# samson6460/tf2_YOLO

Measured on AMD Instinct MI355X. Metric: images/sec training YOLOv3 416x416 bs=32/GPU, higher is better.
Workload: dtype f32-storage/fp16x2-mfma

## Files before the change

### include/yolo_hip.h

```cpp
#ifndef YOLO_HIP_H_
#define YOLO_HIP_H_

#include <stddef.h>
#include <stdint.h>

#ifdef __cplusplus
extern "C" {
#endif

typedef enum yolo_status {
  YOLO_OK = 0,
  YOLO_ERR_INVALID_ARG = -1,
  YOLO_ERR_LAUNCH = -2,
  YOLO_ERR_WORKSPACE = -3
} yolo_status;

enum { YOLO_ACT_LINEAR = 0, YOLO_ACT_LEAKY = 1, YOLO_ACT_MISH = 2 };
enum { YOLO_HEAD_V3 = 3, YOLO_HEAD_V2 = 2, YOLO_HEAD_V1 = 1, YOLO_HEAD_V4 = 4 };
enum { YOLO_NMS_HARD = 1, YOLO_NMS_SOFT = 2, YOLO_NMS_DIOU = 3 };

const char* yolo_last_error(void);
int yolo_abi_version(void);
int yolo_device_available(void);
int yolo_mfma_probe(const void* operands_f16, float* sink, int workgroups, int iters, double* flops_host, void* stream);

enum { YOLO_OPT_CONV_WIN = 0, YOLO_OPT_STAMPS = 1, YOLO_OPT_CONV_SK = 2, YOLO_OPT_CONV_PATCH = 5, YOLO_OPT_WGRAD_WIN = 6,
       YOLO_OPT_NMS_WALK = 7 ,
       YOLO_OPT_AB = 8  };
int yolo_set_option(int key, int value);
size_t yolo_conv_workspace_bytes(void);
int yolo_set_conv_workspace(void* p, size_t bytes, void* stream);
int yolo_set_debug_buffer(void* p, size_t bytes);

typedef struct yolo_conv_desc {
  int N, H, W, Cin;
  int Cout, kh, kw;
  int Ho, Wo;
  int sh, sw;
  int pad_t, pad_l;
} yolo_conv_desc;

#define YOLO_BN_STAT_SLOTS 64
#define YOLO_BN_RED_SLOTS 512
#define YOLO_SPLIT_BATCH_UNITS 4

int yolo_conv2d_fwd(const yolo_conv_desc* d, const float* x, const float* w,
                    const float* bias, float* y, double* stats, void* stream);
int yolo_conv2d_fwd_absmax(const yolo_conv_desc* d, const float* x, const float* w, const float* bias,
                           float* y, double* stats, unsigned* absmax, void* stream);

int yolo_conv2d_dgrad(const yolo_conv_desc* d, const float* dy, const float* wT,
                      float* dx, int accumulate, void* stream);

int yolo_conv2d_wgrad(const yolo_conv_desc* d, const float* x, const float* dy,
                      float* dw, float* dbias, void* stream);

int yolo_conv2d_wgrad_bias(const float* dy, long long P, int Cout, float* dbias, void* stream);

int yolo_filter_transpose(const float* w, float* wT, int Cout, int taps, int Cin, void* stream);

size_t yolo_planes_bytes(long long rows, int C);
int yolo_split_planes(const float* x, long long rows, int C, void* planes, void* stream);
int yolo_split_planes_padded(const float* x, long long rows, int C_src, int C, void* planes, void* stream);

int yolo_split_planes_batch(const void* jobs, int njobs, long long total_blocks, void* stream);
int yolo_filter_transpose_batch(const void* jobs, int njobs, long long total_blocks, void* stream);

int yolo_conv2d_fwd_planes(const yolo_conv_desc* d, const void* x_planes, const void* w_planes,
                           const float* bias, float* y, double* stats, unsigned* absmax, void* stream);
int yolo_conv2d_dgrad_planes(const yolo_conv_desc* d, const void* dy_planes, const void* wT_planes,
                             float* dx, int accumulate, void* stream);
enum { YOLO_EPI_NONE = 0, YOLO_EPI_AFFINE = 1, YOLO_EPI_AFFINE_LEAKY = 2, YOLO_EPI_AFFINE_MISH = 3 };
int yolo_conv2d_fwd_planes_epi(const yolo_conv_desc* d, const void* x_planes, const void* w_planes, const float* bias,
                               int epilogue, const float* scale, const float* shift, const float* residual, float* y,
                               unsigned* absmax, void* stream);
int yolo_split_planes_absmax(const float* x, long long rows, int C, const unsigned* absmax, const float* extra_bound,
                             void* planes, float* out_bound, void* stream);
#define YOLO_INFER_BOUND_WORDS 4096
int yolo_conv_pred_bound(const float* w, int Cout, int kdim, const float* scale, const float* shift, const float* bias,
                         float* pred2, void* stream);
int yolo_conv2d_fwd_infer_unit(const yolo_conv_desc* d, const void* x_planes, const void* w_planes, const float* bias,
                               int epilogue, const float* scale, const float* shift, const float* residual, float* y,
                               unsigned* absmax, const float* pred2, const void* in_bound, int in_n,
                               const void* residual_bound, int residual_n, void* out_planes, unsigned* out_words,
                               float* out_bound, int* out_n_host, void* stream);
int yolo_fold_bound(const void* words, int n, float* out_bound, void* stream);
int yolo_absmax_words(const float* x, long long n, unsigned* words, int* n_words_host, void* stream);
int yolo_stem_filter_prep(const float* w, const float* bias, float* wt, void* stream);
int yolo_stem_fwd_infer_unit(const yolo_conv_desc* d, const float* x, const float* wt, int epilogue, const float* scale,
                             const float* shift, const float* pred2, const void* in_bound, int in_n, float* y,
                             void* out_planes, unsigned* out_words, int* out_n_host, void* stream);
int yolo_split_planes_concat(const float* const* srcs_host, const int* channels_host, const float* const* bounds_host,
                             int nsrc, long long rows, void* planes, float* dst32, float* out_bound, void* stream);
int yolo_split_planes_concat_ex(const float* const* srcs_host, const int* channels_host, const float* const* bounds_host,
                                const int* bound_words_host, const int* upsample_host, int H, int W, int nsrc,
                                long long rows, void* planes, float* dst32, float* out_bound, void* stream);
int yolo_conv2d_fwd_head_unit(const yolo_conv_desc* d, const void* x_planes, const void* w_planes, const float* bias,
                              int A, int C, int version, const float* anchors, float* t, float* y, void* stream);
int yolo_conv2d_wgrad_planes(const yolo_conv_desc* d, const void* x_planes, const void* dy_planes,
                             float* dw, void* stream);

size_t yolo_wgrad_workspace_bytes(void);
int yolo_set_wgrad_workspace(void* p, size_t bytes);


int yolo_bn_stats(const float* x, long long P, int C, double* stats, void* stream);

int yolo_bn_finalize(double* stats, long long P, int C, const float* gamma, const float* beta,
                     float eps, float momentum, int unbiased_moving_var,
                     float* moving_mean, float* moving_var,
                     float* scale, float* shift, float* save_mean, float* save_invstd,
// ... 177 lines not shown
```

### tf2_yolo_amd/csrc/conv_args.hpp

```cpp
#pragma once
#include "common.hpp"

namespace yolo {

constexpr int MAX_TAPS = 49;

struct Tap {
  int oy, ox, woff;
};

struct ClassGeom {
  long long M;
  int Hg, Wg, ooy, oox, tap0, ntaps;
};

struct GatherConvArgs {
  const float* src;
  const float* wgt;
  const float* bias;
  float* dst;
  double* stats;
  unsigned* absmax;
  long long M;
  int N, Hs, Ws, Cs;
// ... 22 lines not shown
  const unsigned* pl_res_bound;
  int pl_in_n, pl_res_n;
  unsigned* pl_out_words;
  float* head_y;
  const float* head_anchors;
  int head_A, head_C;
  int sk_grid;
  int tile_order;
  float* sk_slabs;
  unsigned* sk_tickets;
  int split_parts;
  int ncls;
  ClassGeom cls[4];
  unsigned long long* stamps;
  const float* bwd_y;
  const float* bwd_scale;
  const float* bwd_shift;
  const float* bwd_mean;
  const float* bwd_invstd;
  float* bwd_part;
  unsigned* bwd_aux;
  int bwd_act;
  int bwd_nslots;
  int bwd_cap;
  Tap taps[MAX_TAPS];
};

#define YOLO_BNRED_CHECK(a)                                                                                          \
  if ((a).bwd_y != nullptr && (a).bwd_nslots > (a).bwd_cap) {                                                        \
    set_error("conv_dgrad(bn reduce): %d partial slots needed, room for %d", (a).bwd_nslots, (a).bwd_cap);           \
    return YOLO_ERR_INVALID_ARG;                                                                                     \
  }

__device__ __forceinline__ int xcd_remap(int bid, int nblocks) {
  const int xcd = bid & 7, idx = bid >> 3;
  const int q = nblocks >> 3, r = nblocks & 7;
  const int start = (xcd < r) ? xcd * (q + 1) : r * (q + 1) + (xcd - r) * q;
  return start + idx;
}


struct WgradArgs {
  const float* src;
  const float* dy;
  float* dw;
  long long M;
  int N, Hs, Ws, Cs;
  int Hg, Wg;
  int sy, sx;
  int Cout, ldw;
  int ntaps;
  int kw, pad_t, pad_l;
  int tiles_co, tiles_j;
  int nblocks;
  long long chunk;
  unsigned src_bytes, dy_bytes;
  int zero_blk_src, zero_blk_dy;
  float* slabs;
  int splits;
};

int launch_gather_split(GatherConvArgs& a, hipStream_t st);
bool gather_split_supported(const GatherConvArgs& a);
long long planes_bytes(long long rows, int C);
int launch_split_planes(const float* x, long long rows, int C, void* planes, hipStream_t st);
int launch_split_planes_absmax(const float* x, long long rows, int C, const unsigned* absmax, const float* extra_bound, int extra_n,
                               void* planes, float* out_bound, hipStream_t st);
int launch_split_planes_concat(const float* const* xs, const int* Cs, const float* const* bounds, int nsrc, long long rows,
                               void* planes, float* dst32, float* out_bound, hipStream_t st,
                               const int* bound_words = nullptr, const int* upsample = nullptr, int H = 0, int W = 0);
int launch_split_planes_padded(const float* x, long long rows, int Csrc, int C, void* planes, hipStream_t st);
int launch_split_planes_batch(const void* jobs, int njobs, long long total_blocks, hipStream_t st);
int launch_filter_transpose_batch(const void* jobs, int njobs, long long total_blocks, hipStream_t st);
int launch_gather_planes(GatherConvArgs& a, hipStream_t st);
bool conv_small_supported(const GatherConvArgs& a);
bool conv_small_head_supported(const GatherConvArgs& a);
int launch_conv_small(GatherConvArgs& a, hipStream_t st, int* nwg);
bool gather_planes_supported(const GatherConvArgs& a);
int conv_split_parts(const GatherConvArgs& a, long long nb, int bm, int min_cb, int idle_div);
int launch_split_reduce(GatherConvArgs& a, int bm, hipStream_t st);
float* conv_split_slabs();
int launch_conv_win(GatherConvArgs& a, int variant, hipStream_t st);
bool conv_win_supported(const GatherConvArgs& a);
enum { OPT_CONV_WIN = 0, OPT_STAMPS = 1, OPT_CONV_SK = 2, OPT_DBG = 3, OPT_TILE_ORDER = 4, OPT_CONV_PATCH = 5, OPT_WGRAD_WIN = 6, OPT_NMS_WALK = 7, OPT_EXP = 8, OPT_COUNT = 16 };
int set_conv_workspace(void* p, size_t bytes, hipStream_t st);
extern void* g_dbg_buf;
extern size_t g_dbg_bytes;
extern int g_opt[OPT_COUNT];
void init_options();
int launch_wgrad_planes(WgradArgs& a, hipStream_t st);
bool wgrad_planes_supported(const WgradArgs& a);
int launch_wgrad_win(WgradArgs& a, hipStream_t st);
bool wgrad_win_supported(const WgradArgs& a);
constexpr size_t WGRAD_WS_COLSUM_BYTES = 1 << 20;
void* wgrad_workspace(size_t* bytes);
bool stem_fwd_supported(const yolo_conv_desc* d);
struct StemEpiArgs {
  const float* scale;
  const float* shift;
  int act;
  void* planes;
  const float* pred;
  const unsigned* in_words;
  int in_n;
  unsigned* out_words;
};
bool stem_infer_supported(const yolo_conv_desc* d);
int launch_stem_filter_prep(const float* w, const float* bias, float* wt, hipStream_t st);
int launch_absmax_words(const float* x, long long n, unsigned* words, int* n_words, hipStream_t st);
int launch_stem_infer(const yolo_conv_desc* d, const float* x, const float* wt, float* y, const StemEpiArgs& e, int* out_n,
                      hipStream_t st);
size_t stem_bwd_scratch_bytes();
int launch_stem_bn_bwd_wgrad(const yolo_conv_desc* d, const float* y, const float* dout, const float* img, const float* scale,
                             const float* shift, const float* smean, const float* sinv, int act, const double* redsum,
                             float* dgamma, float* dbeta, float* dw, float* scratch, size_t scratch_bytes, hipStream_t st);
int launch_stem_fwd(const yolo_conv_desc* d, const float* x, const float* w, const float* bias, float* y, double* stats,
                    unsigned* absmax, hipStream_t st);
int launch_wgrad_split(WgradArgs& a, hipStream_t st);
bool wgrad_split_supported(const WgradArgs& a);

}
```

### tf2_yolo_amd/csrc/conv_wgrad_win.hip

```cpp
#include "planes.hpp"
#include <cstdlib>

namespace yolo {

typedef short ws16x4 __attribute__((ext_vector_type(4)));
typedef short ws16x8 __attribute__((ext_vector_type(8)));

constexpr int WW_CO = 128;
constexpr int WW_CI = 32;
constexpr int WW_STAGE_PX = 32;
constexpr int WW_TILE_FLOATS = WW_CO * 9 * WW_CI;

template <int RING, int KO = 0, int PF = 1>
__global__ __launch_bounds__(256, 2) void wgrad_win_kernel(const WgradArgs a) {
  constexpr int A_STAGE = 2 * 4 * PL_PLANES * 1024;
  constexpr int WIN_PLANE = RING * 64 + 64;
  constexpr int WIN_OFF = 2 * A_STAGE;
  constexpr unsigned RMASK = RING * 64 - 1;
  constexpr unsigned ZSLOT = RING * 64;

  extern __shared__ __attribute__((aligned(16))) unsigned char smem[];
  const unsigned lds_base = (unsigned)(size_t)smem;

  const int tid = threadIdx.x;
// ... 645 lines not shown
        acc[t][hf][1] = __builtin_amdgcn_mfma_f32_16x16x32_f16(ah[1], bh[cur], acc[t][hf][1], 0, 0, 0);
      }
      __builtin_amdgcn_sched_barrier(0);
      if (i == 17) {
#pragma unroll
        for (int r = 0; r < 2; ++r) {
          pb[r] = (pb[r] + WW_STAGE_PX * 64) & RMASK;
          int x = px[r] + adv_rem, y = py[r] + adv_rows;
          if (x >= W) {
            x -= W;
            ++y;
          }
          if (y >= H) y -= H;
          px[r] = x;
          py[r] = y;
        }
        __builtin_amdgcn_sched_barrier(0);
      }
    }
    asm volatile("s_waitcnt vmcnt(0)" ::: "memory");
    asm volatile("s_waitcnt lgkmcnt(0)" ::: "memory");
    __builtin_amdgcn_s_barrier();
  }

  const float unscale =
      reinterpret_cast<const float*>(reinterpret_cast<const unsigned char*>(a.dy) + a.dy_bytes - PL_HEADER)[2] *
      reinterpret_cast<const float*>(reinterpret_cast<const unsigned char*>(a.src) + a.src_bytes - PL_HEADER)[2];
  if (a.slabs != nullptr) {
    float* mine = a.slabs + (size_t)lid * WW_TILE_FLOATS;
#pragma unroll
    for (int t = 0; t < 9; ++t)
#pragma unroll
      for (int hf = 0; hf < 2; ++hf)
#pragma unroll
        for (int m = 0; m < 2; ++m)
          *reinterpret_cast<f32x4*>(mine + (((((wave * 9 + t) * 2 + hf) * 2 + m) * 64) + lane) * 4) = acc[t][hf][m];
    return;
  }
#pragma unroll
  for (int t = 0; t < 9; ++t)
#pragma unroll
    for (int hf = 0; hf < 2; ++hf) {
      const long long cj = (long long)t * a.Cs + ci0 + 16 * hf + (lane & 15);
#pragma unroll
      for (int m = 0; m < 2; ++m)
#pragma unroll
        for (int e = 0; e < 4; ++e) {
          const int co = co0 + wave * 32 + 16 * m + 4 * (lane >> 4) + e;
          atomicAdd(&a.dw[(long long)co * a.ldw + cj], acc[t][hf][m][e] * unscale);
        }
    }
}

__global__ __launch_bounds__(256) void wgrad_win16_reduce_kernel(const WgradArgs a) {
  constexpr int PER_TILE = WW_TILE_FLOATS / 4;
  const int tiles = a.tiles_co * a.tiles_j;
  const long long idx = (long long)blockIdx.x * 256 + threadIdx.x;
  const int tile = (int)(idx / PER_TILE);
  if (tile >= tiles) return;
  const int q = (int)(idx - (long long)tile * PER_TILE);
  const int lane = q & 63, piece = q >> 6;
  const int m = piece & 1, hf = (piece >> 1) & 1, t = (piece >> 2) % 9, wave = piece / 36;
  const int co = (tile % a.tiles_co) * WW_CO + wave * 32 + 16 * m + 4 * (lane >> 4);
  const long long cj = (long long)t * a.Cs + (tile / a.tiles_co) * WW_CI + 16 * hf + (lane & 15);
  const f32x4* sl = reinterpret_cast<const f32x4*>(a.slabs) + (size_t)tile * PER_TILE + q;
  const size_t sstride = (size_t)tiles * PER_TILE;
  f32x4 sum = {0.f, 0.f, 0.f, 0.f};
  int s = 0;
  for (; s + 8 <= a.splits; s += 8) {
    f32x4 v[8];
#pragma unroll
    for (int u = 0; u < 8; ++u) v[u] = __builtin_nontemporal_load(sl + (size_t)(s + u) * sstride);
#pragma unroll
    for (int u = 0; u < 8; ++u) sum = sum + v[u];
  }
  for (; s < a.splits; ++s) sum = sum + __builtin_nontemporal_load(sl + (size_t)s * sstride);
  const float unscale =
      reinterpret_cast<const float*>(reinterpret_cast<const unsigned char*>(a.dy) + a.dy_bytes - PL_HEADER)[2] *
      reinterpret_cast<const float*>(reinterpret_cast<const unsigned char*>(a.src) + a.src_bytes - PL_HEADER)[2];
#pragma unroll
  for (int e = 0; e < 4; ++e) a.dw[(long long)(co + e) * a.ldw + cj] += sum[e] * unscale;
}

bool wgrad_win_supported(const WgradArgs& a) {
  if (a.ntaps != 9 || a.kw != 3 || a.sy != 1 || a.sx != 1 || a.pad_t != 1 || a.pad_l != 1) return false;
  if (a.Hg != a.Hs || a.Wg != a.Ws) return false;
  if ((a.Cout % WW_CO) != 0 || (a.Cs % WW_CI) != 0 || a.ldw != 9 * a.Cs) return false;
  if (a.Ws < 4 || 2 * a.Ws + 81 > 512 || 32 / a.Ws + 2 > a.Hs) return false;
  if (a.M < 64 || a.M >= (1LL << 31) - 4096) return false;
  return true;
}

template <int RING, int KO, int PF = 1, bool M16 = false>
static int launch_ww(WgradArgs& a, hipStream_t st) {
  const void* kfn = M16 ? reinterpret_cast<const void*>(&wgrad_win16_kernel<RING, KO>)
                        : reinterpret_cast<const void*>(&wgrad_win_kernel<RING, KO, PF>);
  a.tiles_co = a.Cout / WW_CO;
  a.tiles_j = a.Cs / WW_CI;
  const long long tiles = (long long)a.tiles_co * a.tiles_j;
  constexpr size_t lds = 2 * (2 * 4 * PL_PLANES * 1024) + 2 * (RING * 64 + 64);
  static int resident = 0;
  static bool lds_from_zero = true;
  if (resident == 0) {
    int per_cu = 0, dev = 0, cus = 0;
    hipFuncAttributes fa{};
    if (hipFuncGetAttributes(&fa, kfn) != hipSuccess || fa.sharedSizeBytes != 0) lds_from_zero = false;
    (void)hipFuncSetAttribute(kfn, hipFuncAttributeMaxDynamicSharedMemorySize, (int)lds);
    if (hipOccupancyMaxActiveBlocksPerMultiprocessor(&per_cu, kfn, 256, lds) ==
            hipSuccess &&
        hipGetDevice(&dev) == hipSuccess && hipDeviceGetAttribute(&cus, hipDeviceAttributeMultiprocessorCount, dev) == hipSuccess)
      resident = per_cu * cus;
    if (resident <= 0) resident = 512;
  }
  if (!lds_from_zero) return 1;
  static const long long target_env = [] { const char* e = getenv("YOLO_WGRAD_WIN_TARGET"); return e ? atoll(e) : 0LL; }();
  const long long target = target_env > 0 ? target_env : (resident >= 2 ? resident / 2 : resident);
  long long splits = target / tiles;
  const long long max_splits = (a.M + 255) / 256;
  if (splits > max_splits) splits = max_splits;
  if (splits < 1) splits = 1;
  a.slabs = nullptr;
  static const bool det_env = [] { const char* e = getenv("YOLO_WGRAD_DETERMINISTIC"); return !(e && atoi(e) == 0); }();
  size_t ws_bytes = 0;
  void* ws = wgrad_workspace(&ws_bytes);
  if (det_env && ws != nullptr && ws_bytes > WGRAD_WS_COLSUM_BYTES) {
    const long long cap = (long long)((ws_bytes - WGRAD_WS_COLSUM_BYTES) / ((size_t)WW_TILE_FLOATS * 4));
    if (cap >= tiles) {
      if (tiles * splits > cap) splits = cap / tiles;
      a.slabs = reinterpret_cast<float*>(reinterpret_cast<unsigned char*>(ws) + WGRAD_WS_COLSUM_BYTES);
    }
  }
  long long chunk = (a.M + splits - 1) / splits;
  chunk = (chunk + 31) / 32 * 32;
  splits = (a.M + chunk - 1) / chunk;
  a.chunk = chunk;
  a.splits = (int)splits;
  a.nblocks = (int)(tiles * splits);
  if constexpr (M16) hipLaunchKernelGGL((wgrad_win16_kernel<RING, KO>), dim3((unsigned)a.nblocks), dim3(256), lds, st, a);
  else hipLaunchKernelGGL((wgrad_win_kernel<RING, KO, PF>), dim3((unsigned)a.nblocks), dim3(256), lds, st, a);
  if (int rc = check_launch("wgrad_win_kernel")) return rc;
  if (a.slabs != nullptr) {
    const long long pieces = tiles * (WW_TILE_FLOATS / 4);
    if constexpr (M16) hipLaunchKernelGGL(wgrad_win16_reduce_kernel, dim3((unsigned)((pieces + 255) / 256)), dim3(256), 0, st, a);
    else hipLaunchKernelGGL(wgrad_win_reduce_kernel, dim3((unsigned)((pieces + 255) / 256)), dim3(256), 0, st, a);
    return check_launch("wgrad_win_reduce_kernel");
  }
  return YOLO_OK;
}

static int launch_ww2(WgradArgs& a, hipStream_t st) {
  constexpr int RING = 256;
  const void* kfn = reinterpret_cast<const void*>(&wgrad_win2_kernel<RING>);
  a.tiles_co = a.Cout / WW_CO;
  a.tiles_j = a.Cs / WW_CI;
  const long long tiles = (long long)a.tiles_co * a.tiles_j;
  constexpr size_t half_bytes = 2 * (2 * 4 * PL_PLANES * 1024) + 2 * (RING * 64 + 64);
  constexpr size_t handover = (size_t)WW_TILE_FLOATS * 4;
  constexpr size_t lds = 2 * half_bytes > handover ? 2 * half_bytes : handover;
  static int resident = 0;
  static bool ok = true;
  if (resident == 0) {
    int per_cu = 0, dev = 0, cus = 0;
    hipFuncAttributes fa{};
    if (hipFuncGetAttributes(&fa, kfn) != hipSuccess || fa.sharedSizeBytes != 0) ok = false;
    if (hipFuncSetAttribute(kfn, hipFuncAttributeMaxDynamicSharedMemorySize, (int)lds) != hipSuccess) ok = false;
    if (hipOccupancyMaxActiveBlocksPerMultiprocessor(&per_cu, kfn, 512, lds) == hipSuccess && per_cu >= 1 &&
        hipGetDevice(&dev) == hipSuccess && hipDeviceGetAttribute(&cus, hipDeviceAttributeMultiprocessorCount, dev) == hipSuccess)
      resident = per_cu * cus;
    else
      ok = false;
    if (resident <= 0) resident = 256;
  }
  if (!ok) return 1;
  size_t ws_bytes = 0;
  void* ws = wgrad_workspace(&ws_bytes);
  static const bool det_env = [] { const char* e = getenv("YOLO_WGRAD_DETERMINISTIC"); return !(e && atoi(e) == 0); }();
  if (!det_env || ws == nullptr || ws_bytes <= WGRAD_WS_COLSUM_BYTES) return 1;
  long long splits = resident / tiles;
  const long long max_splits = (a.M + 511) / 512;
  if (splits > max_splits) splits = max_splits;
  if (splits < 1) splits = 1;
  const long long cap = (long long)((ws_bytes - WGRAD_WS_COLSUM_BYTES) / ((size_t)WW_TILE_FLOATS * 4));
  if (cap < tiles) return 1;
  if (tiles * splits > cap) splits = cap / tiles;
  a.slabs = reinterpret_cast<float*>(reinterpret_cast<unsigned char*>(ws) + WGRAD_WS_COLSUM_BYTES);
  long long chunk = (a.M + splits - 1) / splits;
  chunk = (chunk + 63) / 64 * 64;
  splits = (a.M + chunk - 1) / chunk;
  a.chunk = chunk;
  a.splits = (int)splits;
  a.nblocks = (int)(tiles * splits);
  hipLaunchKernelGGL((wgrad_win2_kernel<RING>), dim3((unsigned)a.nblocks), dim3(512), lds, st, a);
  if (int rc = check_launch("wgrad_win2_kernel")) return rc;
  const long long pieces = tiles * (WW_TILE_FLOATS / 4);
  hipLaunchKernelGGL(wgrad_win_reduce_kernel, dim3((unsigned)((pieces + 255) / 256)), dim3(256), 0, st, a);
  return check_launch("wgrad_win_reduce_kernel");
}

int launch_wgrad_win(WgradArgs& a, hipStream_t st) {
  const bool small = 2 * a.Ws + 81 <= 256;
  if (small && g_opt[OPT_WGRAD_WIN] == 4) {
    const int rc = launch_ww2(a, st);
    if (rc != 1) return rc;
  }
#ifdef YOLO_PLANES_KNOCKOUTS
  static const int ko = [] { const char* e = getenv("YOLO_WGRAD_KO"); return e ? atoi(e) : 0; }();
  if (small) switch (ko) {
      case 1: return launch_ww<256, 1>(a, st);
      case 2: return launch_ww<256, 2>(a, st);
      case 3: return launch_ww<256, 3>(a, st);
      case 4: return launch_ww<256, 4>(a, st);
      case 7: return launch_ww<256, 7>(a, st);
      case 8: return launch_ww<256, 8>(a, st);
      default: break;
    }
#endif
  if (small && g_opt[OPT_WGRAD_WIN] == 2) return launch_ww<256, 0, 2>(a, st);
  if (g_opt[OPT_WGRAD_WIN] == 3) return small ? launch_ww<256, 0, 1, true>(a, st) : launch_ww<512, 0, 1, true>(a, st);
  return small ? launch_ww<256, 0>(a, st) : launch_ww<512, 0>(a, st);
}

}
```

### tf2_yolo_amd/csrc/runtime.hip

```cpp
#include "conv_args.hpp"
#include <cstdlib>
#include <cstring>

namespace yolo {

static thread_local char g_err[512] = "";

void set_error(const char* fmt, ...) {
  va_list ap;
  va_start(ap, fmt);
  vsnprintf(g_err, sizeof(g_err), fmt, ap);
  va_end(ap);
}

int g_opt[OPT_COUNT];
void* g_dbg_buf = nullptr;
size_t g_dbg_bytes = 0;
static void options_from_env() {
  for (int i = 0; i < OPT_COUNT; ++i) g_opt[i] = 0;
  const char* e = getenv("YOLO_CONV_WIN");
  g_opt[OPT_CONV_WIN] = e ? atoi(e) : 1;
  e = getenv("YOLO_CONV_SK");
  g_opt[OPT_CONV_SK] = e ? atoi(e) : 1;
  e = getenv("YOLO_CONV_PATCH");
  g_opt[OPT_CONV_PATCH] = e ? atoi(e) : 1;
  e = getenv("YOLO_WGRAD_WIN");
  g_opt[OPT_WGRAD_WIN] = e ? atoi(e) : 1;
  e = getenv("YOLO_NMS_WALK");
  g_opt[OPT_NMS_WALK] = e ? atoi(e) : 0;
  e = getenv("YOLO_EXP");
  g_opt[OPT_EXP] = e ? atoi(e) : 0;
}
void init_options() {
  static bool done = false;
  if (done) return;
  done = true;
  options_from_env();
}

}

extern "C" int yolo_set_option(int key, int value) {
  yolo::init_options();
  if (key == -1) {
    yolo::options_from_env();
    return YOLO_OK;
  }
  if (key < 0 || key >= yolo::OPT_COUNT) {
    yolo::set_error("yolo_set_option: unknown key %d", key);
    return YOLO_ERR_INVALID_ARG;
  }
  yolo::g_opt[key] = value;
  return YOLO_OK;
}

extern "C" size_t yolo_conv_workspace_bytes(void) { return (size_t)(1 << 20) + (size_t)512 * 2 * 256 * 128 * 4; }

extern "C" int yolo_set_conv_workspace(void* p, size_t bytes, void* stream) {
  yolo::init_options();
  return yolo::set_conv_workspace(p, bytes, yolo::as_stream(stream));
}

extern "C" int yolo_set_debug_buffer(void* p, size_t bytes) {
  yolo::g_dbg_buf = p;
  yolo::g_dbg_bytes = bytes;
  return YOLO_OK;
}

extern "C" const char* yolo_last_error(void) { return yolo::g_err; }

extern "C" int yolo_abi_version(void) { return 5; }

#include <dlfcn.h>
namespace {
using nccl_allreduce_fn = int (*)(const void*, void*, size_t, int, int, void*, hipStream_t);
nccl_allreduce_fn find_nccl_allreduce() {
  void* f = dlsym(RTLD_DEFAULT, "ncclAllReduce");
  if (f == nullptr) {
    void* h = dlopen("librccl.so.1", RTLD_NOW | RTLD_GLOBAL);
    if (h == nullptr) h = dlopen("librccl.so", RTLD_NOW | RTLD_GLOBAL);
    if (h != nullptr) f = dlsym(h, "ncclAllReduce");
  }
  return reinterpret_cast<nccl_allreduce_fn>(f);
}
}

extern "C" int yolo_allreduce_bucket(void* rccl_comm, float* grads, long long count, void* stream) {
  YOLO_REQUIRE(rccl_comm != nullptr && grads != nullptr && count > 0, "allreduce_bucket: bad args");
  static nccl_allreduce_fn fn = find_nccl_allreduce();
  if (fn == nullptr) {
    yolo::set_error("allreduce_bucket: no RCCL in this process (ncclAllReduce not found, librccl.so not loadable)");
    return YOLO_ERR_LAUNCH;
  }
  constexpr int kNcclFloat = 7, kNcclSum = 0;
  const int rc = fn(grads, grads, (size_t)count, kNcclFloat, kNcclSum, rccl_comm, yolo::as_stream(stream));
  if (rc != 0) {
    yolo::set_error("allreduce_bucket: ncclAllReduce returned %d", rc);
    return YOLO_ERR_LAUNCH;
  }
  return YOLO_OK;
}

extern "C" int yolo_device_available(void) {
  int n = 0;
  if (hipGetDeviceCount(&n) != hipSuccess) return 0;
  return n > 0 ? 1 : 0;
}
```

### tf2_yolo_amd/ops.py

```python
import ctypes
from ctypes import byref, c_void_p

import torch

from . import _lib
from . import tape as _tape
from ._lib import ConvDesc, LossCfg, YoloHipError, check

BN_EPS = 1e-3
BN_MOMENTUM = 0.99
BN_STAT_SLOTS = 64
BN_RED_SLOTS = 512
SPLIT_BATCH_UNITS = 4


class KernelTimer:

    def __init__(self):
        self.pending = []

    def bracket(self, name, flops, launches, fn, layer=None):
        s, e = torch.cuda.Event(enable_timing=True), torch.cuda.Event(enable_timing=True)
        s.record()
        fn()
        e.record()
        self.pending.append((name, flops, launches, s, e, layer))

    def summary(self, by_layer=False):
        torch.cuda.synchronize()
        agg = {}
        for name, flops, launches, s, e, layer in self.pending:
            a = agg.setdefault((name, layer) if by_layer else name, {"launches": 0, "ms": 0.0, "flops": 0.0})
            a["launches"] += launches
            a["ms"] += s.elapsed_time(e)
            a["flops"] += flops
        self.pending = []
        return agg


TIMER = None


def _conv_flops(d):
    return 2.0 * d.N * d.Ho * d.Wo * d.Cout * d.kh * d.kw * d.Cin


def _layer_key(d, which):
    return (which, d.H, d.W, d.Cin, d.Cout, d.kh, d.sh, d.N)


import os as _os
CONV_MODE = "fp32" if _os.environ.get("YOLO_CONV_MODE", "split")[:1] in ("f", "0") else "split"
USE_PLANES = CONV_MODE == "split" and _os.environ.get("YOLO_CONV_PLANES", "1") != "0"


def planes_fwd_ok(cin, cout):
    return USE_PLANES and cin % 16 == 0 and cout >= 32


def planes_dgrad_ok(cin, cout):
    return USE_PLANES and cout % 16 == 0 and cin >= 32


def planes_wgrad_ok(cin, cout, taps, stride=1):
    return USE_PLANES and cin % 16 == 0 and cout % 16 == 0 and cout >= 32 and taps * cin >= 64


_WGRAD_WIDE = int(_os.environ.get("YOLO_WGRAD_WIDE", "2"))


WGRAD_WIN = int(_os.environ.get("YOLO_WGRAD_WIN", "1"))


def _wgrad_win_covers(d):
    m = d.N * d.Ho * d.Wo
    return (WGRAD_WIN != 0 and d.kh == 3 and d.kw == 3 and d.sh == 1 and d.sw == 1 and d.pad_t == 1 and d.pad_l == 1
            and d.H == d.Ho and d.W == d.Wo and d.Cout % 128 == 0 and d.Cin % 32 == 0 and d.W >= 4
            and 2 * d.W + 81 <= 512 and 32 // d.W + 2 <= d.H and 64 <= m < (1 << 31) - 4096)


def _wgrad_planes_variant(cout, cols, taps=1, pixels=1 << 40, d=None):
    if d is not None and _wgrad_win_covers(d):
        return "wgrad_win_planes_kernel<128,288%s>" % (",mfma16" if WGRAD_WIN == 3 else "")
    if cout > 64 and cols >= 256 and (_WGRAD_WIDE == 1 or (_WGRAD_WIDE == 2 and taps > 1 and pixels <= 8192)):
        return "wgrad_planes_kernel<128,256,2,2>"
    big = "4,2" if _os.environ.get("YOLO_WGRAD_WAVES") == "8" else "2,2"
    return "wgrad_planes_kernel<%d,%d,%s>" % (64 if cout <= 64 else 128, 64 if cols <= 64 else 128,
                                             "2,2" if (cout <= 64 and cols <= 64) else "2,4" if cout <= 64
                                             else "4,2" if cols <= 64 else big)


_PLANES_WAVES = int(_os.environ.get("YOLO_PLANES_WAVES", "0") or 0)


CONV_WIN = int(_os.environ.get("YOLO_CONV_WIN", "1"))
CONV_PATCH = int(_os.environ.get("YOLO_CONV_PATCH", "1"))


def _planes_variant(cout, win=None, k1=False):
    if win is not None and CONV_WIN not in (0, 2, 4) and CONV_PATCH and cout >= 64:
        ws, m, hs, n = win
        narrow = cout <= 64
        tiles = (n * ((hs + 15) // 16) * ((ws + 15) // 16) if narrow
                 else n * ((hs + 7) // 8) * ((ws + 15) // 16) * ((cout + 127) // 128))
        if CONV_PATCH == 2 or ((narrow or ws > 64) and tiles >= 256):
            return "conv_patch_planes_kernel<%s>" % ("256,64" if narrow else "128,128")
    if win is not None and CONV_WIN and cout >= 128:
        ws, m = win[:2]
        wgm = CONV_WIN if CONV_WIN in (2, 4) else (0 if ws > 64 else 2)
        if wgm:
            return "conv_win_planes_kernel<%d,128>" % (64 * wgm)
    if cout <= 32:
        return "gather_conv_planes_kernel<128,32,4,1>"
    if cout <= 64:
        return "gather_conv_planes_kernel<128,64,4,2>"
    waves8 = _PLANES_WAVES == 8 or (_PLANES_WAVES == 0 and k1)
    return "gather_conv_planes_kernel<128,128,%s>" % ("4,2" if waves8 else "2,2")


def _win_key(d, hs, ws, cs):
    if d.kh == 3 and d.kw == 3 and d.sh == 1 and d.sw == 1 and d.pad_t == 1 and d.pad_l == 1 and cs % 16 == 0 \
            and d.H == d.Ho and d.W == d.Wo:
        return (ws, d.N * hs * ws, hs, d.N)
    return None


def _gather_variant(cout, flat, m=None):
    bn = 32 if cout <= 32 else (64 if cout <= 64 else 128)
    bm = 128
    if bn == 128 and not flat and m is not None and ((m + 127) // 128) * ((cout + 127) // 128) <= 512:
        bm = 64
    if CONV_MODE == "split" and not flat and cout > 32:
        waves = {(128, 64): "2,2", (64, 128): "1,4", (128, 128): "4,2"}[(bm, bn)]
        return f"gather_conv_split_kernel<{bm},{bn},{waves}>"
    return f"gather_conv_kernel<{bm},{bn}{',flat' if flat else ''}>"


OPT_CONV_WIN = 0
OPT_CONV_SK = 2
OPT_CONV_PATCH = 5
OPT_WGRAD_WIN = 6
OPT_NMS_WALK = 7
_CONV_WS = None


def ensure_conv_workspace():
    global _CONV_WS
    if _CONV_WS is not None and _CONV_WS.device.index != torch.cuda.current_device():
        raise YoloHipError(f"libyolo_hip.so was initialised on cuda:{_CONV_WS.device.index} and cannot also serve "
                           f"cuda:{torch.cuda.current_device()}: start one process per GPU")
    if _CONV_WS is None:
        lib = _lib.load()
        n = int(lib.yolo_conv_workspace_bytes())
        _CONV_WS = torch.empty(n, dtype=torch.uint8, device="cuda")
        check(lib.yolo_set_conv_workspace(_p(_CONV_WS), n, _stream()), "yolo_set_conv_workspace")
    return _CONV_WS


_WGRAD_WS = None


def ensure_wgrad_workspace():
    global _WGRAD_WS
    if _WGRAD_WS is None:
        lib = _lib.load()
        n = int(lib.yolo_wgrad_workspace_bytes())
        _WGRAD_WS = torch.empty(n, dtype=torch.uint8, device="cuda")
        check(lib.yolo_set_wgrad_workspace(_p(_WGRAD_WS), n), "yolo_set_wgrad_workspace")
    return _WGRAD_WS


_SIDE_STREAMS = {}


def _overlaps(a, b, cycles=6000000):
    e0, e1, e2 = (torch.cuda.Event(enable_timing=True) for _ in range(3))
    torch.cuda.synchronize()
    with torch.cuda.stream(a):
        e0.record(a)
        torch.cuda._sleep(cycles)
        e1.record(a)
    torch.cuda.synchronize()
    one = e0.elapsed_time(e1)
    with torch.cuda.stream(a):
        e0.record(a)
    b.wait_event(e0)
    with torch.cuda.stream(b):
        torch.cuda._sleep(cycles)
    with torch.cuda.stream(a):
        torch.cuda._sleep(cycles)
    a.wait_stream(b)
    e2.record(a)
    torch.cuda.synchronize()
    return e0.elapsed_time(e2) < 1.5 * one


def create_side_streams(device=None):
    dev = torch.cuda.current_device() if device is None else torch.device(device).index
    if dev is None:
        dev = torch.cuda.current_device()
    for role in ("wgrad", "comm"):
        if (dev, role) not in _SIDE_STREAMS:
            st = torch.cuda.Stream(device=dev)
            if (_os.environ.get("YOLO_STREAM_PROBE") == "1" and dev == torch.cuda.current_device()
                    and not _overlaps(torch.cuda.current_stream(), st)):
                import warnings
                warnings.warn(f"tf2_yolo_amd: the {role} stream shares a hardware queue with the compute stream: the step "
                              "will run them one after the other (create_side_streams() earlier, or raise GPU_MAX_HW_QUEUES)")
            _SIDE_STREAMS[(dev, role)] = st
    return {role: _SIDE_STREAMS[(dev, role)] for role in ("wgrad", "comm")}


def concurrent_stream(role, beside=None, device=None):
    st = create_side_streams(device)[role]
    want = torch.cuda.current_device() if device is None else torch.device(device).index
    if want is not None and st.device.index != want:
        raise YoloHipError(f"side stream of role {role!r} lives on cuda:{st.device.index}, not on cuda:{want}")
    return st


def set_option(key, value):
    global WGRAD_WIN
    check(_lib.load().yolo_set_option(int(key), int(value)), "yolo_set_option")
    if int(key) == OPT_WGRAD_WIN:
        WGRAD_WIN = int(value)


def reset_options():
    global WGRAD_WIN
    check(_lib.load().yolo_set_option(-1, 0), "yolo_set_option")
    WGRAD_WIN = int(_os.environ.get("YOLO_WGRAD_WIN", "1"))


def _stream():
    return c_void_p(torch.cuda.current_stream().cuda_stream)


def _p(t):
    if t is None:
        return c_void_p(0)
    if _tape.ACTIVE is not None:
        _tape.ACTIVE.keep.append(t)
    return c_void_p(t.data_ptr())


def _chk_f32(*ts):
    for t in ts:
        if t is None:
            continue
        if not (t.is_cuda and t.dtype == torch.float32 and t.is_contiguous()):
            raise YoloHipError("expected a contiguous float32 CUDA tensor, got "
                               f"{t.dtype} {t.device} contiguous={t.is_contiguous()}")


def same_pad(size, k, s):
    out = -(-size // s)
    total = max((out - 1) * s + k - size, 0)
    return out, total // 2


def conv_desc(x_shape, cout, kh, kw, stride, padding):
    n, h, w, cin = x_shape
    if padding == "same":
        ho, pt = same_pad(h, kh, stride)
        wo, pl = same_pad(w, kw, stride)
    elif padding == "valid":
        ho, wo, pt, pl = (h - kh) // stride + 1, (w - kw) // stride + 1, 0, 0
    elif padding == "darknet_s2":
        ho, wo, pt, pl = (h + 1 - kh) // stride + 1, (w + 1 - kw) // stride + 1, 1, 1
    else:
        raise ValueError(f"bad padding {padding}")
    return ConvDesc(n, h, w, cin, cout, kh, kw, ho, wo, stride, stride, pt, pl)


def conv2d_fwd(d, x, w, bias=None, out=None, stats=None, absmax=None):
    _chk_f32(x, w, bias)
    if out is None:
        out = torch.empty((d.N, d.Ho, d.Wo, d.Cout), device=x.device, dtype=torch.float32)
    if x.numel() != d.N * d.H * d.W * d.Cin or w.numel() != d.Cout * d.kh * d.kw * d.Cin:
        raise YoloHipError("conv2d_fwd: tensor sizes do not match the descriptor")
    if out.numel() != d.N * d.Ho * d.Wo * d.Cout:
        raise YoloHipError("conv2d_fwd: output size does not match the descriptor")
    if stats is not None and stats.numel() != BN_STAT_SLOTS * 2 * d.Cout:
        raise YoloHipError("conv2d_fwd: stats must hold BN_STAT_SLOTS x 2 x Cout doubles")
    def run():
        check(_lib.load().yolo_conv2d_fwd_absmax(byref(d), _p(x), _p(w), _p(bias), _p(out), _p(stats), _p(absmax),
                                                 _stream()), "yolo_conv2d_fwd")
    if TIMER is not None:
        stem = (CONV_MODE == "split" and _os.environ.get("YOLO_STEM_DIRECT", "1") != "0" and d.Cin == 3 and d.Cout == 32
                and d.kh == 3 and d.kw == 3 and d.sh == 1 and d.sw == 1 and d.Ho == d.H and d.Wo == d.W
                and d.N * d.H * d.W >= (1 << 20))
        name = "stem_conv3x3_kernel" if stem else _gather_variant(d.Cout, d.Cin % 32 != 0, d.N * d.Ho * d.Wo)
        TIMER.bracket(name, _conv_flops(d), 1, run)
    else:
        run()
    return out


def planes_bytes(rows, c):
    n = int(_lib.load().yolo_planes_bytes(int(rows), int(c)))
    if n == 0:
        raise YoloHipError(f"planes: unsupported shape rows={rows} C={c} (C must be a multiple of 16)")
    return n


def split_planes(x, rows, c, out=None):
    _chk_f32(x)
    if x.numel() != rows * c:
        raise YoloHipError("split_planes: tensor size does not match rows x C")
    n = planes_bytes(rows, c)
    if out is None:
        out = torch.empty(n, device=x.device, dtype=torch.uint8)
    elif out.numel() < n or out.dtype != torch.uint8:
        raise YoloHipError("split_planes: output buffer too small")
# ... 855 lines not shown
```

Before: 1066.

## Add 64-wide Cout windowed wgrad kernel for 3x3 convs with Cout not divisible by 128

Adds a windowed weight-gradient kernel for 3x3 stride-1 convolutions whose output-channel count is a multiple of 64 but not of 128, such as 64-channel layers. These previously fell back to the generic planes wgrad path. The kernel keeps a sliding LDS ring of input pixels and issues three fp16 MFMAs per tap, writing split-K partial slabs that a separate reduce kernel sums into dw. It is enabled by default through a new option, and it adds a second launch plus a slab round trip through the workspace.

```diff
diff --git a/include/yolo_hip.h b/include/yolo_hip.h
--- a/include/yolo_hip.h
+++ b/include/yolo_hip.h
@@ -26,7 +26,8 @@
 
 enum { YOLO_OPT_CONV_WIN = 0, YOLO_OPT_STAMPS = 1, YOLO_OPT_CONV_SK = 2, YOLO_OPT_CONV_PATCH = 5, YOLO_OPT_WGRAD_WIN = 6,
        YOLO_OPT_NMS_WALK = 7 ,
-       YOLO_OPT_AB = 8  };
+       YOLO_OPT_AB = 8 ,
+       YOLO_OPT_WGRAD_WIN64 = 9  };
 int yolo_set_option(int key, int value);
 size_t yolo_conv_workspace_bytes(void);
 int yolo_set_conv_workspace(void* p, size_t bytes, void* stream);
diff --git a/tf2_yolo_amd/csrc/conv_args.hpp b/tf2_yolo_amd/csrc/conv_args.hpp
--- a/tf2_yolo_amd/csrc/conv_args.hpp
+++ b/tf2_yolo_amd/csrc/conv_args.hpp
@@ -128,7 +128,7 @@
 float* conv_split_slabs();
 int launch_conv_win(GatherConvArgs& a, int variant, hipStream_t st);
 bool conv_win_supported(const GatherConvArgs& a);
-enum { OPT_CONV_WIN = 0, OPT_STAMPS = 1, OPT_CONV_SK = 2, OPT_DBG = 3, OPT_TILE_ORDER = 4, OPT_CONV_PATCH = 5, OPT_WGRAD_WIN = 6, OPT_NMS_WALK = 7, OPT_EXP = 8, OPT_COUNT = 16 };
+enum { OPT_CONV_WIN = 0, OPT_STAMPS = 1, OPT_CONV_SK = 2, OPT_DBG = 3, OPT_TILE_ORDER = 4, OPT_CONV_PATCH = 5, OPT_WGRAD_WIN = 6, OPT_NMS_WALK = 7, OPT_EXP = 8, OPT_WGRAD_WIN64 = 9, OPT_COUNT = 16 };
 int set_conv_workspace(void* p, size_t bytes, hipStream_t st);
 extern void* g_dbg_buf;
 extern size_t g_dbg_bytes;
diff --git a/tf2_yolo_amd/csrc/conv_wgrad_win.hip b/tf2_yolo_amd/csrc/conv_wgrad_win.hip
--- a/tf2_yolo_amd/csrc/conv_wgrad_win.hip
+++ b/tf2_yolo_amd/csrc/conv_wgrad_win.hip
@@ -751,13 +751,288 @@
   for (int e = 0; e < 4; ++e) a.dw[(long long)(co + e) * a.ldw + cj] += sum[e] * unscale;
 }
 
+constexpr int W64_CO = 64;
+template <int RING, int NBUF>
+__global__ __launch_bounds__(256, 1) void wgrad_win64_kernel(const WgradArgs a) {
+  constexpr int PF = 1;
+  constexpr int A_STAGE = 2 * 2 * PL_PLANES * 1024;
+  constexpr int WIN_PLANE = RING * 64 + 64;
+  constexpr int WIN_OFF = NBUF * A_STAGE;
+  constexpr unsigned RMASK = RING * 64 - 1;
+  constexpr unsigned ZSLOT = RING * 64;
+
+  extern __shared__ __attribute__((aligned(16))) unsigned char smem[];
+  const unsigned lds_base = (unsigned)(size_t)smem;
+
+  const int tid = threadIdx.x;
+  const int lane = tid & 63;
+  const int wave = __builtin_amdgcn_readfirstlane(tid >> 6);
+  const int fb = wave & 1, kj = wave >> 1;
+
+  const int lid = xcd_remap(blockIdx.x, a.nblocks);
+  const int tiles = a.tiles_co * a.tiles_j;
+  const int split = lid / tiles;
+  const int tile = lid - split * tiles;
+  const int co0 = (tile % a.tiles_co) * W64_CO;
+  const int ci0 = (tile / a.tiles_co) * WW_CI;
+  const int p_begin = (int)((long long)split * a.chunk);
+  int p_end = p_begin + (int)a.chunk;
+  if (p_end > (int)a.M) p_end = (int)a.M;
+  if (p_begin >= p_end) return;
+  const int nst = (p_end - p_begin + WW_STAGE_PX - 1) / WW_STAGE_PX;
+  const int W = a.Ws, H = a.Hs, M = (int)a.M;
+
+  if (tid < 32) reinterpret_cast<unsigned*>(smem + WIN_OFF + (tid >> 4) * WIN_PLANE + ZSLOT)[tid & 15] = 0u;
+
+  const unsigned strideA = (unsigned)((a.Cout >> 4) * PL_RECORD);
+  const unsigned strideB = (unsigned)((a.Cs >> 4) * PL_RECORD);
+  const unsigned zeroA = (unsigned)a.zero_blk_dy * strideA, zeroB = (unsigned)a.zero_blk_src * strideB;
+  const i32x4 rsrcA = planes_rsrc(a.dy, a.dy_bytes), rsrcB = planes_rsrc(a.src, a.src_bytes);
+  const int lpix = 4 * (lane >> 4) + (lane & 3), lsb = (lane >> 2) & 3;
+  const unsigned a_lane = (unsigned)(((co0 + fb * 32) >> 4) + (lsb >> 1)) * PL_RECORD + (lsb & 1) * 256 + lpix * 16;
+  const unsigned a_piece = (unsigned)((kj * 2 + fb) * PL_PLANES * 1024);
+  auto issue_A = [&](int stage) {
+    const int pb16 = p_begin + stage * WW_STAGE_PX + kj * 16;
+    const unsigned v = (pb16 < p_end) ? (unsigned)(pb16 >> 4) * strideA + a_lane : zeroA;
+#pragma unroll
+    for (int p = 0; p < PL_PLANES; ++p) {
+      const unsigned l = __builtin_amdgcn_readfirstlane(lds_base + (stage % NBUF) * A_STAGE + a_piece + p * 1024);
+      dma16(rsrcA, v, (unsigned)(p * 512), l);
+    }
+  };
+  const int bpx = lane >> 2, bch = lane & 3;
+  const unsigned b_lane = (unsigned)((ci0 >> 4) + (bch >> 1)) * PL_RECORD + (bch & 1) * 256;
+  auto issue_B = [&](int P0, int plane) {
+    const int P = P0 + bpx;
+    const unsigned v = ((unsigned)P < (unsigned)M) ? (unsigned)(P >> 4) * strideB + b_lane + (P & 15) * 16 : zeroB;
+    const unsigned l = __builtin_amdgcn_readfirstlane(lds_base + WIN_OFF + plane * WIN_PLANE + (unsigned)((P0 & (RING - 1)) * 64));
+    dma16(rsrcB, v, (unsigned)(plane * 512), l);
+  };
+
+  const int lo = (p_begin - W - 1) & ~15;
+  const int Lbase = (p_begin + W + 33 + 15) & ~15;
+  {
+    const int npieces = ((Lbase - lo) >> 4) * PL_PLANES;
+    for (int idx = wave; idx < npieces; idx += 4) issue_B(lo + (idx >> 1) * 16, idx & 1);
+  }
+#pragma unroll
+  for (int s = 0; s < NBUF - 1; ++s) issue_A(s);
+
+  const int grp = lane >> 4, i16 = lane & 15;
+  const int qq = i16 >> 2, pq = i16 & 3;
+  const int tr_off = ((2 * (grp >> 1)) * 16 + ((grp & 1) * 2 + (pq >> 1)) * 4 + qq) * 16 + (pq & 1) * 8;
+  const unsigned lc = (unsigned)((2 * (grp & 1) + (pq >> 1)) * 16 + (pq & 1) * 8);
+  typedef ws16x4 __attribute__((address_space(3))) * lds_p;
+  unsigned pb[2];
+  int px[2], py[2];
+#pragma unroll
+  for (int r = 0; r < 2; ++r) {
+    const int p = p_begin + 16 * kj + 8 * (grp >> 1) + 4 * r + qq;
+    pb[r] = (((unsigned)p & (RING - 1)) << 6) + lc;
+    const int row = p / W;
+    px[r] = p - row * W;
+    py[r] = row % H;
+  }
+  const int adv_rows = WW_STAGE_PX / W, adv_rem = WW_STAGE_PX - adv_rows * W;
+  int shb[9];
+#pragma unroll
+  for (int t = 0; t < 9; ++t) shb[t] = ((t / 3 - 1) * W + (t % 3 - 1)) * 64;
+
+  f32x16 acc[9];
+#pragma unroll
+  for (int t = 0; t < 9; ++t)
+#pragma unroll
+    for (int q = 0; q < 16; ++q) acc[t][q] = 0.f;
+
+  asm volatile("s_waitcnt vmcnt(0) lgkmcnt(0)" ::: "memory");
+  __builtin_amdgcn_s_barrier();
+
+  auto rd_pair = [&](unsigned a0, unsigned a1, int off) -> f16x8 {
+    const ws16x4 v0 = __builtin_amdgcn_ds_read_tr16_b64_v4i16((lds_p)(size_t)(a0 + off));
+    const ws16x4 v1 = __builtin_amdgcn_ds_read_tr16_b64_v4i16((lds_p)(size_t)(a1 + off));
+    const ws16x8 v = {v0[0], v0[1], v0[2], v0[3], v1[0], v1[1], v1[2], v1[3]};
+    return __builtin_bit_cast(f16x8, v);
+  };
+  const unsigned zl = ZSLOT + lc;
+  for (int s = 0; s < nst; ++s) {
+    issue_B(Lbase + s * WW_STAGE_PX + (wave >> 1) * 16, wave & 1);
+    issue_A(s + NBUF - 1);
+    const unsigned abase = (unsigned)((s % NBUF) * A_STAGE) + a_piece + tr_off;
+    bool okx0[2], okx1[2], oky0[2], oky1[2];
+#pragma unroll
+    for (int r = 0; r < 2; ++r) {
+      okx0[r] = px[r] != 0;
+      okx1[r] = px[r] != W - 1;
+      oky0[r] = py[r] != 0;
+      oky1[r] = py[r] != H - 1;
+    }
+    auto calc = [&](int t, unsigned (&ad)[2]) {
+      const int ty = t / 3, tx = t % 3;
+#pragma unroll
+      for (int r = 0; r < 2; ++r) {
+        bool ok = true;
+        if (ty == 0) ok = ok && oky0[r];
+        if (ty == 2) ok = ok && oky1[r];
+        if (tx == 0) ok = ok && okx0[r];
+        if (tx == 2) ok = ok && okx1[r];
+        const unsigned av = (pb[r] + (unsigned)shb[t]) & RMASK;
+        ad[r] = ok ? av : zl;
+      }
+    };
+    constexpr int NS = PF + 1;
+    f16x8 ah, al, bh[NS], bl[NS];
+    unsigned ad[NS][2];
+#pragma unroll
+    for (int k = 0; k <= PF; ++k) calc(k, ad[k]);
+    ah = rd_pair(abase, abase + 256, 0);
+    al = rd_pair(abase, abase + 256, 1024);
+#pragma unroll
+    for (int k = 0; k < PF; ++k) {
+      bh[k] = rd_pair(ad[k][0], ad[k][1], WIN_OFF);
+      bl[k] = rd_pair(ad[k][0], ad[k][1], WIN_OFF + WIN_PLANE);
+    }
+    __builtin_amdgcn_sched_barrier(0);
+#pragma unroll
+    for (int t = 0; t < 9; ++t) {
+      const int cur = t % NS, nxt = (t + PF) % NS;
+      acc[t] = __builtin_amdgcn_mfma_f32_32x32x16_f16(al, bh[cur], acc[t], 0, 0, 0);
+      __builtin_amdgcn_sched_barrier(0);
+      if (t + PF < 9) {
+        bh[nxt] = rd_pair(ad[nxt][0], ad[nxt][1], WIN_OFF);
+        bl[nxt] = rd_pair(ad[nxt][0], ad[nxt][1], WIN_OFF + WIN_PLANE);
+      }
+      __builtin_amdgcn_sched_barrier(0);
+      acc[t] = __builtin_amdgcn_mfma_f32_32x32x16_f16(ah, bl[cur], acc[t], 0, 0, 0);
+      __builtin_amdgcn_sched_barrier(0);
+      if (t + PF + 1 < 9) calc(t + PF + 1, ad[cur]);
+      __builtin_amdgcn_sched_barrier(0);
+      acc[t] = __builtin_amdgcn_mfma_f32_32x32x16_f16(ah, bh[cur], acc[t], 0, 0, 0);
+      __builtin_amdgcn_sched_barrier(0);
+    }
+#pragma unroll
+    for (int r = 0; r < 2; ++r) {
+      pb[r] = (pb[r] + WW_STAGE_PX * 64) & RMASK;
+      int x = px[r] + adv_rem, y = py[r] + adv_rows;
+      if (x >= W) {
+        x -= W;
+        ++y;
+      }
+      if (y >= H) y -= H;
+      px[r] = x;
+      py[r] = y;
+    }
+    asm volatile("s_waitcnt vmcnt(2)" ::: "memory");
+    asm volatile("s_waitcnt lgkmcnt(0)" ::: "memory");
+    __builtin_amdgcn_s_barrier();
+  }
+  asm volatile("s_waitcnt vmcnt(0)" ::: "memory");
+
+  float* mine = a.slabs + (size_t)lid * WW_TILE_FLOATS;
+#pragma unroll
+  for (int t = 0; t < 9; ++t)
+#pragma unroll
+    for (int q4 = 0; q4 < 4; ++q4) {
+      const f32x4 f = {acc[t][4 * q4], acc[t][4 * q4 + 1], acc[t][4 * q4 + 2], acc[t][4 * q4 + 3]};
+      *reinterpret_cast<f32x4*>(mine + (((wave * 9 + t) * 4 + q4) * 64 + lane) * 4) = f;
+    }
+}
+
+__global__ __launch_bounds__(256) void wgrad_win64_reduce_kernel(const WgradArgs a) {
+  constexpr int PER_TILE = WW_TILE_FLOATS / 4;
+  constexpr int PER_OUT = PER_TILE / 2;
+  const int tiles = a.tiles_co * a.tiles_j;
+  const long long idx = (long long)blockIdx.x * 256 + threadIdx.x;
+  const int tile = (int)(idx / PER_OUT);
+  if (tile >= tiles) return;
+  const int q = (int)(idx - (long long)tile * PER_OUT);
+  const int lane = q & 63, piece = q >> 6;
+  const int q4 = piece & 3, t = (piece >> 2) % 9, fb = piece / 36;
+  const int co = (tile % a.tiles_co) * W64_CO + fb * 32 + 8 * q4 + 4 * (lane >> 5);
+  const long long cj = (long long)t * a.Cs + (tile / a.tiles_co) * WW_CI + (lane & 31);
+  const f32x4* sl = reinterpret_cast<const f32x4*>(a.slabs) + (size_t)tile * PER_TILE + q;
+  const size_t sstride = (size_t)tiles * PER_TILE;
+  f32x4 sum = {0.f, 0.f, 0.f, 0.f};
+  int s = 0;
+  for (; s + 4 <= a.splits; s += 4) {
+    f32x4 v[8];
+#pragma unroll
+    for (int u = 0; u < 4; ++u) {
+      v[2 * u] = __builtin_nontemporal_load(sl + (size_t)(s + u) * sstride);
+      v[2 * u + 1] = __builtin_nontemporal_load(sl + (size_t)(s + u) * sstride + PER_OUT);
+    }
+#pragma unroll
+    for (int u = 0; u < 8; ++u) sum = sum + v[u];
+  }
+  for (; s < a.splits; ++s) {
+    sum = sum + __builtin_nontemporal_load(sl + (size_t)s * sstride);
+    sum = sum + __builtin_nontemporal_load(sl + (size_t)s * sstride + PER_OUT);
+  }
+  const float unscale =
+      reinterpret_cast<const float*>(reinterpret_cast<const unsigned char*>(a.dy) + a.dy_bytes - PL_HEADER)[2] *
+      reinterpret_cast<const float*>(reinterpret_cast<const unsigned char*>(a.src) + a.src_bytes - PL_HEADER)[2];
+#pragma unroll
+  for (int e = 0; e < 4; ++e) a.dw[(long long)(co + e) * a.ldw + cj] += sum[e] * unscale;
+}
+
+static bool wgrad_win64_covers(const WgradArgs& a) {
+  return g_opt[OPT_WGRAD_WIN64] != 0 && (a.Cout % WW_CO) != 0 && (a.Cout % W64_CO) == 0 && 2 * a.Ws + 81 <= 512;
+}
+
 bool wgrad_win_supported(const WgradArgs& a) {
   if (a.ntaps != 9 || a.kw != 3 || a.sy != 1 || a.sx != 1 || a.pad_t != 1 || a.pad_l != 1) return false;
   if (a.Hg != a.Hs || a.Wg != a.Ws) return false;
-  if ((a.Cout % WW_CO) != 0 || (a.Cs % WW_CI) != 0 || a.ldw != 9 * a.Cs) return false;
-  if (a.Ws < 4 || 2 * a.Ws + 81 > 512 || 32 / a.Ws + 2 > a.Hs) return false;
+  if ((a.Cs % WW_CI) != 0 || a.ldw != 9 * a.Cs) return false;
+  if (a.Ws < 4 || 32 / a.Ws + 2 > a.Hs) return false;
   if (a.M < 64 || a.M >= (1LL << 31) - 4096) return false;
-  return true;
+  if (wgrad_win64_covers(a)) return true;
+  return (a.Cout % WW_CO) == 0 && 2 * a.Ws + 81 <= 512;
+}
+
+template <int RING, int NBUF>
+static int launch_ww64(WgradArgs& a, hipStream_t st) {
+  const void* kfn = reinterpret_cast<const void*>(&wgrad_win64_kernel<RING, NBUF>);
+  a.tiles_co = a.Cout / W64_CO;
+  a.tiles_j = a.Cs / WW_CI;
+  const long long tiles = (long long)a.tiles_co * a.tiles_j;
+  constexpr size_t lds = (size_t)NBUF * (2 * 2 * PL_PLANES * 1024) + 2 * (RING * 64 + 64);
+  static_assert(lds <= 160 * 1024, "wgrad_win64_kernel: LDS");
+  static int cus = 0;
+  static bool ok = true;
+  if (cus == 0) {
+    int per_cu = 0, dev = 0;
+    hipFuncAttributes fa{};
+    if (hipFuncGetAttributes(&fa, kfn) != hipSuccess || fa.sharedSizeBytes != 0) ok = false;
+    if (hipFuncSetAttribute(kfn, hipFuncAttributeMaxDynamicSharedMemorySize, (int)lds) != hipSuccess) ok = false;
+    if (hipOccupancyMaxActiveBlocksPerMultiprocessor(&per_cu, kfn, 256, lds) != hipSuccess || per_cu < 1) ok = false;
+    if (hipGetDevice(&dev) != hipSuccess || hipDeviceGetAttribute(&cus, hipDeviceAttributeMultiprocessorCount, dev) != hipSuccess)
+      ok = false;
+    if (cus <= 0) cus = 256;
+  }
+  if (!ok) return 1;
+  size_t ws_bytes = 0;
+  void* ws = wgrad_workspace(&ws_bytes);
+  static const bool det_env = [] { const char* e = getenv("YOLO_WGRAD_DETERMINISTIC"); return !(e && atoi(e) == 0); }();
+  if (!det_env || ws == nullptr || ws_bytes <= WGRAD_WS_COLSUM_BYTES) return 1;
+  const long long cap = (long long)((ws_bytes - WGRAD_WS_COLSUM_BYTES) / ((size_t)WW_TILE_FLOATS * 4));
+  if (cap < tiles) return 1;
+  static const long long target_env = [] { const char* e = getenv("YOLO_WGRAD_WIN_TARGET"); return e ? atoll(e) : 0LL; }();
+  long long splits = (target_env > 0 ? target_env : cus) / tiles;
+  const long long max_splits = (a.M + 255) / 256;
+  if (splits > max_splits) splits = max_splits;
+  if (splits < 1) splits = 1;
+  if (tiles * splits > cap) splits = cap / tiles;
+  a.slabs = reinterpret_cast<float*>(reinterpret_cast<unsigned char*>(ws) + WGRAD_WS_COLSUM_BYTES);
+  long long chunk = (a.M + splits - 1) / splits;
+  chunk = (chunk + 31) / 32 * 32;
+  splits = (a.M + chunk - 1) / chunk;
+  a.chunk = chunk;
+  a.splits = (int)splits;
+  a.nblocks = (int)(tiles * splits);
+  hipLaunchKernelGGL((wgrad_win64_kernel<RING, NBUF>), dim3((unsigned)a.nblocks), dim3(256), lds, st, a);
+  if (int rc = check_launch("wgrad_win64_kernel")) return rc;
+  const long long outs = tiles * (WW_TILE_FLOATS / 8);
+  hipLaunchKernelGGL(wgrad_win64_reduce_kernel, dim3((unsigned)((outs + 255) / 256)), dim3(256), 0, st, a);
+  return check_launch("wgrad_win64_reduce_kernel");
 }
 
 template <int RING, int KO, int PF = 1, bool M16 = false>
@@ -867,6 +1142,7 @@
 }
 
 int launch_wgrad_win(WgradArgs& a, hipStream_t st) {
+  if (wgrad_win64_covers(a)) return launch_ww64<512, 4>(a, st);
   const bool small = 2 * a.Ws + 81 <= 256;
   if (small && g_opt[OPT_WGRAD_WIN] == 4) {
     const int rc = launch_ww2(a, st);
diff --git a/tf2_yolo_amd/csrc/runtime.hip b/tf2_yolo_amd/csrc/runtime.hip
--- a/tf2_yolo_amd/csrc/runtime.hip
+++ b/tf2_yolo_amd/csrc/runtime.hip
@@ -28,6 +28,8 @@
   g_opt[OPT_WGRAD_WIN] = e ? atoi(e) : 1;
   e = getenv("YOLO_NMS_WALK");
   g_opt[OPT_NMS_WALK] = e ? atoi(e) : 0;
+  e = getenv("YOLO_WGRAD_WIN64");
+  g_opt[OPT_WGRAD_WIN64] = e ? atoi(e) : 1;
   e = getenv("YOLO_EXP");
   g_opt[OPT_EXP] = e ? atoi(e) : 0;
 }
diff --git a/tf2_yolo_amd/ops.py b/tf2_yolo_amd/ops.py
--- a/tf2_yolo_amd/ops.py
+++ b/tf2_yolo_amd/ops.py
@@ -72,14 +72,24 @@
 WGRAD_WIN = int(_os.environ.get("YOLO_WGRAD_WIN", "1"))
 
 
+WGRAD_WIN64 = int(_os.environ.get("YOLO_WGRAD_WIN64", "1"))
+
+
+def _wgrad_win64_covers(d):
+    return WGRAD_WIN64 != 0 and d.Cout % 128 != 0 and d.Cout % 64 == 0 and 2 * d.W + 81 <= 512
+
+
 def _wgrad_win_covers(d):
     m = d.N * d.Ho * d.Wo
     return (WGRAD_WIN != 0 and d.kh == 3 and d.kw == 3 and d.sh == 1 and d.sw == 1 and d.pad_t == 1 and d.pad_l == 1
-            and d.H == d.Ho and d.W == d.Wo and d.Cout % 128 == 0 and d.Cin % 32 == 0 and d.W >= 4
-            and 2 * d.W + 81 <= 512 and 32 // d.W + 2 <= d.H and 64 <= m < (1 << 31) - 4096)
+            and d.H == d.Ho and d.W == d.Wo and d.Cin % 32 == 0 and d.W >= 4
+            and 32 // d.W + 2 <= d.H and 64 <= m < (1 << 31) - 4096
+            and (_wgrad_win64_covers(d) or (d.Cout % 128 == 0 and 2 * d.W + 81 <= 512)))
 
 
 def _wgrad_planes_variant(cout, cols, taps=1, pixels=1 << 40, d=None):
+    if d is not None and _wgrad_win_covers(d) and _wgrad_win64_covers(d):
+        return "wgrad_win64_kernel<64,288>"
     if d is not None and _wgrad_win_covers(d):
         return "wgrad_win_planes_kernel<128,288%s>" % (",mfma16" if WGRAD_WIN == 3 else "")
     if cout > 64 and cols >= 256 and (_WGRAD_WIDE == 1 or (_WGRAD_WIDE == 2 and taps > 1 and pixels <= 8192)):
@@ -140,6 +150,7 @@
 OPT_CONV_SK = 2
 OPT_CONV_PATCH = 5
 OPT_WGRAD_WIN = 6
+OPT_WGRAD_WIN64 = 9
 OPT_NMS_WALK = 7
 _CONV_WS = None
 
@@ -220,16 +231,19 @@
 
 
 def set_option(key, value):
-    global WGRAD_WIN
+    global WGRAD_WIN, WGRAD_WIN64
     check(_lib.load().yolo_set_option(int(key), int(value)), "yolo_set_option")
     if int(key) == OPT_WGRAD_WIN:
         WGRAD_WIN = int(value)
+    if int(key) == OPT_WGRAD_WIN64:
+        WGRAD_WIN64 = int(value)
 
 
 def reset_options():
-    global WGRAD_WIN
+    global WGRAD_WIN, WGRAD_WIN64
     check(_lib.load().yolo_set_option(-1, 0), "yolo_set_option")
     WGRAD_WIN = int(_os.environ.get("YOLO_WGRAD_WIN", "1"))
+    WGRAD_WIN64 = int(_os.environ.get("YOLO_WGRAD_WIN64", "1"))
 
 
 def _stream():
```

New measurement: 1069, median of 6. About the same (+0.3%).
